# braun-steven/DAFNe

Hardware: AMD Instinct MI355X
Metric: images/sec on 1024x1024 DOTA tiles, R101-FPN (higher is better)
Workload: dtype bf16; 1 GPU; DOTA-1.0 1024x1024 R101-FPN bf16, batch 8 per GPU (per-GPU shard of configs[2]; the model BASELINE.json's metric names), uint8 tiles resident in HBM -> detections; per_gpu_batch=8, global_batch=8, classes=15, parallelism=dp1 (independent images, RCCL gather of detections), mode=pipelined

## Files before the change

### dafne_amd/_lib.py

```python
import ctypes
import os

_HERE = os.path.dirname(os.path.abspath(__file__))
LIB_PATH = os.environ.get("DAFNE_AMD_LIB") or os.path.join(_HERE, "libdafne_amd.so")
_lib = None

c_void_p = ctypes.c_void_p
c_int = ctypes.c_int
c_i64 = ctypes.c_int64
c_size_t = ctypes.c_size_t
c_double = ctypes.c_double
c_float = ctypes.c_float
c_u32 = ctypes.c_uint32
c_i32 = ctypes.c_int32


class LevelDesc(ctypes.Structure):
    _fields_ = [("d_logits", c_void_p), ("d_delta", c_void_p), ("d_center", c_void_p),
                ("d_ctrness", c_void_p), ("logits_ps", c_i32), ("delta_ps", c_i32),
                ("center_ps", c_i32), ("ctrness_ps", c_i32), ("H", c_i32), ("W", c_i32), ("stride", c_i32),
                ("scale", c_float)]


class DecodeParams(ctypes.Structure):
# ... 95 lines not shown
    "dafne_conv2d_wr_workspace_bytes": (c_size_t, [ctypes.POINTER(ConvParams), ctypes.POINTER(ConvSeg)]),
    "dafne_conv2d_wr_hip": (c_int, [ctypes.POINTER(ConvParams), ctypes.POINTER(ConvSeg), c_void_p, c_void_p, c_size_t, c_void_p]),
    "dafne_bottleneck_body_scratch_bytes": (c_size_t, []),
    "dafne_bottleneck_body_hip": (c_int, [c_void_p, c_void_p, c_void_p, c_void_p, c_void_p, c_void_p, c_int, c_int, c_int,
                                          c_void_p, c_void_p, c_void_p, c_size_t, c_void_p]),
    "dafne_bottleneck_tail_head_hip": (c_int, [c_void_p, c_void_p, c_void_p, c_void_p, c_void_p, c_int, c_int, c_int,
                                               c_void_p, c_void_p, c_void_p]),
    "dafne_bottleneck_tail_head_narrow_hip": (c_int, [c_void_p, c_void_p, c_void_p, c_void_p, c_void_p, c_int, c_int, c_int,
                                                      c_void_p, c_void_p, c_void_p]),
    "dafne_bottleneck_tail_head_mid_hip": (c_int, [c_void_p, c_void_p, c_void_p, c_void_p, c_void_p, c_int, c_int, c_int,
                                                   c_void_p, c_void_p, c_void_p]),
    "dafne_bottleneck_proj_tail_head_narrow_hip": (c_int, [c_void_p, c_void_p, c_void_p, c_void_p, c_void_p, c_void_p, c_int,
                                                           c_int, c_int, c_void_p, c_void_p, c_void_p]),
    "dafne_bottleneck_block_narrow_scratch_bytes": (c_size_t, []),
    "dafne_bottleneck_block_narrow_hip": (c_int, [c_void_p] * 7 + [c_int, c_int, c_int, c_void_p, c_void_p, c_void_p, c_size_t, c_void_p]),
    "dafne_bottleneck_block_mid_scratch_bytes": (c_size_t, []),
    "dafne_bottleneck_block_mid_hip": (c_int, [c_void_p] * 6 + [c_int, c_int, c_int, c_void_p, c_void_p, c_void_p, c_size_t, c_void_p]),
    "dafne_stem_pool_hip": (c_int, [c_void_p, c_void_p, c_void_p, c_int, c_int, c_int, c_void_p, c_void_p]),
    "dafne_stem_pool_conv1_hip": (c_int, [c_void_p, c_void_p, c_void_p, c_void_p, c_void_p, c_int, c_int, c_int, c_void_p, c_void_p,
                                          c_void_p]),
    "dafne_maxpool3x3s2_nhwc_bf16_hip": (c_int, [c_void_p, c_void_p, c_int, c_int, c_int, c_int, c_void_p]),
    "dafne_groupnorm_relu_nhwc_bf16_hip": (c_int, [ctypes.POINTER(GnSeg), c_int, c_int, c_int, c_void_p, c_void_p,
                                                   c_void_p, c_void_p, c_float, c_void_p]),
    "dafne_relu_copy_bf16_hip": (c_int, [c_void_p, c_void_p, c_i64, c_void_p]),
    "dafne_scene_tiles_workspace_bytes": (c_size_t, [c_int]),
    "dafne_scene_tiles_u8_hip": (c_int, [ctypes.POINTER(SceneTile), c_int, c_int, c_void_p, c_void_p, c_size_t, c_void_p]),
    "dafne_scene_merge_workspace_bytes": (c_size_t, [c_int, c_int]),
    "dafne_scene_merge_rows_hip": (c_int, [c_void_p, c_void_p, c_int, c_int, c_void_p, c_int, c_int, ctypes.c_uint64, c_int,
                                           c_int, c_void_p, c_void_p, c_void_p, c_void_p, c_size_t, c_void_p]),
    "dafne_scene_views_workspace_bytes": (c_size_t, [ctypes.POINTER(ViewSrc), c_int, c_int, c_int]),
# ... 48 lines not shown
```

### dafne_amd/csrc/abi.hip

```cpp
#include "common.h"

namespace dafne {
char* err_buf() {
    static thread_local char buf[512] = {0};
    return buf;
}
}

extern "C" {
int dafne_abi_version(void) { return 145; }
const char* dafne_last_error(void) { return dafne::err_buf(); }
}
```

### dafne_amd/csrc/conv_wr.hip

```cpp
#include <type_traits>

#include "common.h"

namespace {

typedef __attribute__((ext_vector_type(8))) __bf16 bf16x8;
typedef __attribute__((ext_vector_type(16))) float f32x16;
typedef __attribute__((ext_vector_type(4))) float f32x4;
typedef __attribute__((ext_vector_type(4))) unsigned u32x4;
typedef __attribute__((ext_vector_type(2))) unsigned u32x2;
typedef __attribute__((address_space(1))) void gvoid;
typedef __attribute__((address_space(3))) void lvoid;

constexpr int kPx = 128, kCT = 256;
constexpr int kNominalBatch = 8;
constexpr int kNW = 8, kNT = 512;
constexpr int kPF = kPx / 32;
constexpr int kStage = kPx * 128;
constexpr int kNS = 3;
constexpr int kSlabY = kPx * 128;
constexpr int kOffFlag = 4 * kSlabY;
constexpr int kSmemTotal = kOffFlag + 64;
constexpr int kSlabBytes = kPx * kCT * 4;
constexpr int kCounterBytes = 64 * 1024;
// ... 25 lines not shown
    typedef __attribute__((ext_vector_type(2))) float f32x2;
    typedef __attribute__((ext_vector_type(2))) __bf16 bf16x2;
    f32x2 v = {a, b};
    bf16x2 r = __builtin_convertvector(v, bf16x2);
    return __builtin_bit_cast(unsigned, r);
}

template <int I, int N, class F>
__device__ __forceinline__ void static_for(F&& f) {
    if constexpr (I < N) {
        f(std::integral_constant<int, I>{});
        static_for<I + 1, N>(f);
    }
}

__global__ void __launch_bounds__(512, 2) conv_wr_kernel(WrDev P) {
    extern __shared__ __attribute__((aligned(16))) char lds[];
    const int tid = threadIdx.x;
    const int lane = tid & 63;
    const int wave = __builtin_amdgcn_readfirstlane(tid >> 6);
    const int frow = lane & 31, half = lane >> 5;
    const unsigned lds_base = (unsigned)(size_t)(__attribute__((address_space(3))) char*)lds;

    const int id = xcd_remap(blockIdx.x, gridDim.x);
    const int slice = id % P.S;
    const int t = id / P.S;
    const int pt = t % P.ptiles, ct = t / P.ptiles;
    const int k_begin = (int)((long long)slice * P.nsteps / P.S);
    const int k_end = (int)((long long)(slice + 1) * P.nsteps / P.S);
    const int nst = k_end - k_begin;
// ... 82 lines not shown
        const int nxt = cur == kNS - 1 ? 0 : cur + 1;
        static_for<0, 4>([&](auto SS) {
            constexpr int s = decltype(SS)::value;
            if constexpr (s < 3) {
                asm volatile("s_waitcnt vmcnt(11)" : "+v"(ar[par * 4 + s]) :: "memory");
                bread(cur, s + 1, bfr[(s + 1) & 1]);
                asm volatile("s_waitcnt lgkmcnt(4)" : "+v"(bfr[s & 1][0]), "+v"(bfr[s & 1][1]), "+v"(bfr[s & 1][2]), "+v"(bfr[s & 1][3]) :: "memory");
            } else {
                asm volatile("s_waitcnt vmcnt(9)" : "+v"(ar[par * 4 + s]) :: "memory");
                asm volatile("s_waitcnt lgkmcnt(0)" : "+v"(bfr[1][0]), "+v"(bfr[1][1]), "+v"(bfr[1][2]), "+v"(bfr[1][3]) :: "memory");
                __builtin_amdgcn_sched_barrier(0);
                __builtin_amdgcn_s_barrier();
                __builtin_amdgcn_sched_barrier(0);
                bread(nxt, 0, bfr[0]);
            }
            __builtin_amdgcn_sched_barrier(0);
#pragma unroll
            for (int b = 0; b < kPF; b++) acc[b] = __builtin_amdgcn_mfma_f32_32x32x16_bf16(ar[par * 4 + s], bfr[s & 1][b], acc[b], 0, 0, 0);
            __builtin_amdgcn_sched_barrier(0);
            issue_W(4 * i + 8 + s, ar[par * 4 + s]);
            if constexpr (s == 3) issue_P(i + 3, cur);
        });
        cur = nxt;
    };
    int i = 0;
    for (; i + 1 < nst; i += 2) {
        step(i, std::integral_constant<int, 0>{});
        step(i + 1, std::integral_constant<int, 1>{});
    }
    if (i < nst) step(i, std::integral_constant<int, 0>{});
// ... 94 lines not shown
            int img, oy, ox;
            out_coords(px, img, oy, ox);
            char* dst = P.out + (((size_t)(img * (P.Hout + 2) + oy + 1) * (P.Wout + 2) + ox + 1) * P.Cout + ct * kCT) * 2 + q * 16;
#pragma unroll
            for (int sl = 0; sl < 4; sl++) {
                const u32x4 v = *(const u32x4*)(lds + sl * kSlabY + px * 128 + ((q ^ ((px >> 1) & 7)) * 16));
                *(u32x4*)(dst + sl * 128) = v;
            }
        }
    }
}

int wr_build(WrDev& D, const dafne_conv_params* prm, const dafne_conv_seg* segs, const char** why) {
    *why = nullptr;
    if (!prm || !segs) { *why = "null argument"; return 0; }
    const unsigned allowed = DAFNE_CONV_RELU | DAFNE_CONV_RESIDUAL | DAFNE_CONV_UPSAMPLE_ADD | DAFNE_CONV_EXCLUSIVE;
    if (prm->n_segs != 1) { *why = "one segment"; return 0; }
    if (prm->flags & ~allowed) { *why = "flags"; return 0; }
    if ((prm->flags & DAFNE_CONV_RESIDUAL) && (prm->flags & DAFNE_CONV_UPSAMPLE_ADD)) { *why = "residual and top-down add"; return 0; }
    if (!((prm->KH == 1 && prm->KW == 1 && prm->pad == 0) || (prm->KH == 3 && prm->KW == 3 && prm->pad == 1))) { *why = "1x1 p0 or 3x3 p1"; return 0; }
    if (prm->stride != 1 && prm->stride != 2) { *why = "stride"; return 0; }
    if (prm->Cin < 64 || prm->Cin % 64 || prm->Cout < kCT || prm->Cout % kCT) { *why = "Cin % 64, Cout % 256"; return 0; }
    if (!prm->d_bias) { *why = "bias"; return 0; }
    const dafne_conv_seg& S = segs[0];
    if (prm->n_images < 1 || S.Hout < 1 || S.Wout < 1 || (long long)S.Hout * S.Wout > (1 << 20)) { *why = "size"; return 0; }
    if (S.Hout != (S.Hin + 2 * prm->pad - prm->KH) / prm->stride + 1 || S.Wout != (S.Win + 2 * prm->pad - prm->KW) / prm->stride + 1) { *why = "geometry"; return 0; }
    if ((prm->flags & DAFNE_CONV_UPSAMPLE_ADD) && ((S.Hout & 1) || (S.Wout & 1))) { *why = "top-down add on an odd map"; return 0; }
    const long long in_bytes = (long long)prm->n_images * (S.Hin + 2) * (S.Win + 2) * prm->Cin * 2;
    const long long total = (long long)prm->n_images * S.Hout * S.Wout;
    if (in_bytes > 0xffffffffll || total > (1ll << 21)) { *why = "too large"; return 0; }
    D.in = (const char*)S.d_in; D.out = (char*)S.d_out; D.res = (const char*)S.d_res;
// ... 43 lines not shown
}

int dafne_conv2d_wr_hip(const dafne_conv_params* prm, const dafne_conv_seg* segs, const void* d_wfrag, void* d_workspace,
                        size_t workspace_bytes, void* stream) {
    WrDev D;
    const char* why;
    if (!wr_build(D, prm, segs, &why)) return dafne::fail(why && why[0] == 'n' ? DAFNE_E_INVALID : DAFNE_E_UNSUPPORTED, "conv2d_wr: %s", why ? why : "?");
    if (!d_wfrag || !D.in || !D.out) return dafne::fail(DAFNE_E_INVALID, "conv2d_wr: null argument");
    if ((D.flags & (DAFNE_CONV_RESIDUAL | DAFNE_CONV_UPSAMPLE_ADD)) && !D.res) return dafne::fail(DAFNE_E_INVALID, "conv2d_wr: residual flag without d_res");
    const size_t tiles = (size_t)D.ptiles * D.ctiles;
    const size_t need = D.S > 1 ? (size_t)kCounterBytes + tiles * D.S * (size_t)kSlabBytes : 0;
    if (D.S > 1 && (!d_workspace || workspace_bytes < need)) return dafne::fail(DAFNE_E_WORKSPACE, "conv2d_wr: workspace %zu < %zu", workspace_bytes, need);
    D.wf = (const char*)d_wfrag;
    D.counters = (int*)d_workspace;
    D.slabs = (char*)d_workspace + kCounterBytes;
    DAFNE_MAX_LDS_ONCE(kSmemTotal, (const void*)conv_wr_kernel);
    hipLaunchKernelGGL(conv_wr_kernel, dim3((unsigned)(tiles * D.S)), dim3(kNT), kSmemTotal, (hipStream_t)stream, D);
    return dafne::check_launch("conv_wr");
}

}
```

### dafne_amd/engine.py

```python
import ctypes
import os

import torch

from . import _lib

BF16 = torch.bfloat16
STAGE_BLOCKS = {50: (3, 4, 6, 3), 101: (3, 4, 23, 3)}

F_RELU, F_RES, F_UP, F_F32, F_GN, F_GNIN, F_GNFIN, F_EXCL = 1, 2, 4, 8, 16, 32, 64, 128
F_FRAG16 = 256


class Act:

    __slots__ = ("t", "n", "h", "w", "c")

    def __init__(self, n, h, w, c, device):
        self.t = torch.zeros(n, h + 2, w + 2, c, dtype=BF16, device=device)
        self.n, self.h, self.w, self.c = n, h, w, c

    def nchw_float(self):
        return self.t[:, 1:-1, 1:-1, :].permute(0, 3, 1, 2).float().contiguous()

    @staticmethod
    def from_nchw(x):
# ... 492 lines not shown
                if calib is not None:
                    self.calls.append(AmaxProbe(calib, key, [tin]))
                elif key in act_q8:
                    fp8 = (q8[1] / act_q8[key], act_q8[key])
            c = ConvCall(q8[0] if fp8 else wgt, bias, cin, cout, k, stride, pad, flags,
                         [(tin.t, o.t, res.t if res is not None else None, tin.h, tin.w, ho, wo)], n, fp8=fp8,
                         shared_gpu=self.shared_gpu)
            if (fp8 is None and wr_on and wr_takes(k, stride, cin, cout, WR_NOMINAL_BATCH * ho * wo) and bias is not None
                    and L.dafne_conv2d_wr_ok(ctypes.byref(c.prm), c.segs)):
                if key + ".wr" not in P:
                    P[key + ".wr"] = pack_conv_frag(wgt)
                w = WrCall(c, P[key + ".wr"], self.wr_ws)
                self.calls.append(w)
                self.flops += w.flops
                return o
            if fp8 is None and k == 3 and cin == 256 and use_rp_kernel() and c.kernel_id() == 6 and c.rp_ok():
                f16 = rp_frag16()
                fkey = key + (".frag16" if f16 else ".frag")
                if fkey not in P:
                    P[fkey] = pack_rp(wgt)[0]
                c = ConvCall(wgt, bias, cin, cout, k, stride, pad, flags,
                             [(tin.t, o.t, None, tin.h, tin.w, ho, wo)], n, wfrag=P[fkey], shared_gpu=self.shared_gpu, frag16=f16)
            self.calls.append(c)
            self.flops += c.flops
            return o

        self.stem_in = torch.zeros(n, h + 6, w + 6, 4, dtype=BF16, device=device)
        wgt, bias = P["stem"]
        x = pool.get(n, h // 4, w // 4, 64)
        stem_flops = 2 * n * (h // 2) * (w // 2) * 64 * 7 * 7 * 3
# ... 25 lines not shown
            self.calls.append(FnCall(L.dafne_maxpool3x3s2_nhwc_bf16_hip,
                                     (_lib.ptr(stem_out.t), _lib.ptr(x.t), n, h // 2, w // 2, 64),
                                     (stem_out, x), "maxpool"))
            pool.put(stem_out)

        feats = {}
        fuse_b2b = os.environ.get("DAFNE_FUSE_B2B", "1") != "0"
        fuse_narrow = fuse_b2b and os.environ.get("DAFNE_FUSE_B2B_NARROW", "1") != "0"
        fuse_mid = fuse_b2b and os.environ.get("DAFNE_FUSE_B2B_MID", "1") != "0"
        fuse_bneck = fuse_b2b and os.environ.get("DAFNE_FUSE_BNECK", "1") != "0"
        bneck_scratch = None
        blk_scratch = None
        blk_mid_scratch = None
        fuse_blk_mid = fuse_mid and os.environ.get("DAFNE_FUSE_BLK_MID", "1") != "0"
        fuse_blk_narrow = fuse_narrow and os.environ.get("DAFNE_FUSE_BLK_NARROW", "1") != "0"
        for si, nb in enumerate(STAGE_BLOCKS[depth]):
            y1_next = stem_y1 if si == 0 else None
            for b in range(nb):
                p = "res%d.%d." % (si + 2, b)
                stride = 2 if (b == 0 and si > 0) else 1
                w3, b3 = P[p + "conv3"]
                nxt = "res%d.%d.conv1" % (si + 2, b + 1)
                proj_fused = (fuse_narrow and b == 0 and stride == 1 and nb > 1 and tuple(w3.shape) == (256, 64)
                              and tuple(P[p + "shortcut"][0].shape) == (256, 64) and tuple(P[nxt][0].shape) == (64, 256))
                if b == 0:
                    sc = None if proj_fused else conv(p + "shortcut", x, 1, stride, 0, 0)
                else:
                    sc = x
                if y1_next is not None:
                    y1, y1_next = y1_next, None
                else:
                    y1 = conv(p + "conv1", x, 1, stride, 0, F_RELU)
                w2, b2 = P[p + "conv2"]
                q8_2 = P.get(p + "conv2.fp8")
                bn_head = b + 1 < nb
                body_fused = (fuse_bneck and tuple(w3.shape) == (1024, 256) and (not bn_head or tuple(P[nxt][0].shape) == (256, 1024))
                              and (bn_head or os.environ.get("DAFNE_FUSE_BNECK_LAST", "1") != "0")
                              and tuple(w2.shape) == (256, 2304) and y1.c == 256
                              and not (q8_2 is not None and (calib is not None or (p + "conv2") in act_q8)))
                if body_fused:
                    w1, b1 = P[nxt] if bn_head else (torch.zeros(256, 1024, dtype=BF16, device=w2.device), None)
                    key = p + "bneck"
                    if key not in P:
                        P[key] = pack_bneck(w2, w3, w1)
                    if bneck_scratch is None:
                        bneck_scratch = torch.empty(L.dafne_bottleneck_body_scratch_bytes(), dtype=torch.uint8, device=device)
                    inpl = res_dead(sc, x, b)
                    y3 = sc if inpl else pool.get(n, y1.h, y1.w, 1024)
                    y1_next = pool.get(n, y1.h, y1.w, 256) if bn_head else None
                    fl = 2 * n * y1.h * y1.w * (256 * 2304 + 256 * 1024 + (1024 * 256 if bn_head else 0))
                    nb_ = n * y1.h * y1.w * (256 + 1024 + 1024 + (256 if bn_head else 0)) * 2 + (256 * 2304 + 2 * 1024 * 256) * 2
                    self.calls.append(FnCall(L.dafne_bottleneck_body_hip,
                                             (_lib.ptr(y1.t), _lib.ptr(sc.t), _lib.ptr(P[key]), _lib.ptr(b2), _lib.ptr(b3), _lib.ptr(b1),
                                              n, y1.h, y1.w, _lib.ptr(y3.t), _lib.ptr(y1_next.t) if bn_head else None, _lib.ptr(bneck_scratch),
                                              bneck_scratch.numel()),
                                             (y1, sc, P[key], b2, b3, b1, y3, y1_next, bneck_scratch),
                                             "conv_bneck" if bn_head else "conv_bneck_last", flops=fl, nbytes=nb_))
                    self.flops += fl
                    pool.put(y1)
                    if b == 0 and sc is not None and sc is not y3:
                        pool.put(sc)
                    if x is not y3 and not any(x is f for k, f in feats.items() if k != "res2"):
                        pool.put(x)
                    x = y3
                    continue
                if (fuse_blk_narrow and tuple(w2.shape) == (64, 576) and tuple(w3.shape) == (256, 64) and y1.c == 64 and stride == 1
                        and (b > 0 or proj_fused) and (b + 1 >= nb or tuple(P[nxt][0].shape) == (64, 256))):
                    head = b + 1 < nb
                    proj = b == 0
                    w1, b1 = P[nxt] if head else (None, None)
                    wsc, bsc = P[p + "shortcut"] if proj else (None, None)
                    key = p + "blk"
                    if key not in P:
                        P[key] = pack_blk_narrow(w2, w3, w1, wsc)
                    if blk_scratch is None:
                        blk_scratch = torch.empty(L.dafne_bottleneck_block_narrow_scratch_bytes(), dtype=torch.uint8, device=device)
                    src = x if proj else sc
                    inpl = (not proj) and res_dead(sc, x, b)
                    y3 = sc if inpl else pool.get(n, y1.h, y1.w, 256)
                    y1_next = pool.get(n, y1.h, y1.w, 64) if head else None
                    px = n * y1.h * y1.w
                    fl = 2 * px * (64 * 576 + 64 * 256 + (256 * 64 if head else 0) + (64 * 256 if proj else 0))
                    nb_ = px * (64 + (64 if proj else 256) + 256 + (64 if head else 0)) * 2 + P[key].numel() * 2
                    self.calls.append(FnCall(L.dafne_bottleneck_block_narrow_hip,
                                             (_lib.ptr(y1.t), _lib.ptr(src.t), _lib.ptr(P[key]), _lib.ptr(b2), _lib.ptr(b3), _lib.ptr(bsc),
                                              _lib.ptr(b1), n, y1.h, y1.w, _lib.ptr(y3.t), _lib.ptr(y1_next.t) if head else None,
                                              _lib.ptr(blk_scratch), blk_scratch.numel()),
                                             (y1, src, P[key], b2, b3, bsc, b1, y3, y1_next, blk_scratch),
                                             "conv_blk_narrow" + ("_proj" if proj else "") + ("" if head else "_last"), flops=fl, nbytes=nb_))
                    self.flops += fl
                    pool.put(y1)
                    if x is not y3 and not any(x is f for k, f in feats.items() if k != "res2"):
                        pool.put(x)
                    x = y3
                    continue
                if (fuse_blk_mid and tuple(w2.shape) == (128, 1152) and tuple(w3.shape) == (512, 128) and y1.c == 128
                        and (b + 1 >= nb or tuple(P[nxt][0].shape) == (128, 512))):
                    head = b + 1 < nb
                    w1, b1 = P[nxt] if head else (None, None)
                    key = p + "blk"
                    if key not in P:
                        P[key] = pack_blk_mid(w2, w3, w1)
                    if blk_mid_scratch is None:
                        blk_mid_scratch = torch.empty(L.dafne_bottleneck_block_mid_scratch_bytes(), dtype=torch.uint8, device=device)
                    inpl = res_dead(sc, x, b)
                    y3 = sc if inpl else pool.get(n, y1.h, y1.w, 512)
                    y1_next = pool.get(n, y1.h, y1.w, 128) if head else None
                    px = n * y1.h * y1.w
                    fl = 2 * px * (128 * 1152 + 128 * 512 + (512 * 128 if head else 0))
                    nb_ = px * (128 + 512 + 512 + (128 if head else 0)) * 2 + P[key].numel() * 2
                    self.calls.append(FnCall(L.dafne_bottleneck_block_mid_hip,
                                             (_lib.ptr(y1.t), _lib.ptr(sc.t), _lib.ptr(P[key]), _lib.ptr(b2), _lib.ptr(b3), _lib.ptr(b1),
                                              n, y1.h, y1.w, _lib.ptr(y3.t), _lib.ptr(y1_next.t) if head else None,
                                              _lib.ptr(blk_mid_scratch), blk_mid_scratch.numel()),
                                             (y1, sc, P[key], b2, b3, b1, y3, y1_next, blk_mid_scratch),
                                             "conv_blk_mid" + ("" if head else "_last"), flops=fl, nbytes=nb_))
                    self.flops += fl
                    pool.put(y1)
                    if b == 0 and sc is not None and sc is not y3:
                        pool.put(sc)
                    if x is not y3 and not any(x is f for k, f in feats.items() if k != "res2"):
                        pool.put(x)
                    x = y3
                    continue
                y2 = conv(p + "conv2", y1, 3, 1, 1, F_RELU)
                pool.put(y1)
                if proj_fused:
                    w1, b1 = P[nxt]
                    wsc, bsc = P[p + "shortcut"]
                    key = p + "b2b"
                    if key not in P:
                        P[key] = pack_b2b_narrow(w3, w1, wsc)
                    y3 = pool.get(n, y2.h, y2.w, 256)
                    y1_next = pool.get(n, y2.h, y2.w, 64)
                    fl = 2 * n * y2.h * y2.w * (64 * 256 * 2 + 256 * 64)
                    nb_ = n * y2.h * y2.w * (64 + 64 + 256 + 64) * 2 + 3 * 256 * 64 * 2
# ... 37 lines not shown
                        P[key] = pack_b2b_narrow(w3, w1)
                    y3 = pool.get(n, y2.h, y2.w, 256)
                    y1_next = pool.get(n, y2.h, y2.w, 64)
                    fl = 2 * n * y2.h * y2.w * (64 * 256 + 256 * 64)
                    nb_ = n * y2.h * y2.w * (64 + 256 + 256 + 64) * 2 + 2 * 256 * 64 * 2
                    self.calls.append(FnCall(L.dafne_bottleneck_tail_head_narrow_hip,
                                             (_lib.ptr(y2.t), _lib.ptr(sc.t), _lib.ptr(P[key]), _lib.ptr(b3), _lib.ptr(b1),
                                              n, y2.h, y2.w, _lib.ptr(y3.t), _lib.ptr(y1_next.t)),
                                             (y2, sc, P[key], b3, b1, y3, y1_next), "conv_b2b_narrow", flops=fl, nbytes=nb_))
                    self.flops += fl
                else:
                    y3 = conv(p + "conv3", y2, 1, 1, 0, F_RELU | F_RES, res=sc)
                pool.put(y2)
                if b == 0 and sc is not None:
                    pool.put(sc)
                if not any(x is f for k, f in feats.items() if k != "res2"):
                    pool.put(x)
                x = y3
            feats["res%d" % (si + 2)] = x
        self.stage_feats = feats
        prev = None
        outs = {}
        for lvl in (5, 4, 3):
            f = feats["res%d" % lvl]
            lat = conv("fpn_lateral%d" % lvl, f, 1, 1, 0, F_UP if prev is not None else 0, res=prev)
            outs["p%d" % lvl] = conv("fpn_output%d" % lvl, lat, 3, 1, 1, 0)
            prev = lat
        p6 = conv("p6", outs["p5"], 3, 2, 1, 0)
        p6r = pool.get(n, p6.h, p6.w, p6.c)
        self.calls.append(FnCall(L.dafne_relu_copy_bf16_hip, (_lib.ptr(p6.t), _lib.ptr(p6r.t), p6.t.numel()),
                                 (p6, p6r), "relu_copy"))
        p7 = conv("p7", p6r, 3, 2, 1, 0)
        outs["p6"], outs["p7"] = p6, p7
        self.features = [outs[k] for k in ("p3", "p4", "p5", "p6", "p7")]
        self.head_start = len(self.calls)
        self.head = HeadPlan(weights, self.features, num_classes, device, pool, self, head_outputs) if with_head else None
        if any(isinstance(c, WrCall) for c in self.calls):
            self.wr_ws.tensor()

    def run(self, stream=None):
        if self.graph is not None and stream is None:
            self.graph.replay()
            return
        stream = stream if stream is not None else _lib.current_stream()
        for c in self.calls:
            c(stream)

# ... 319 lines not shown
```

### include/dafne_amd.h

```cpp
#ifndef DAFNE_AMD_H
#define DAFNE_AMD_H

#include <stddef.h>
#include <stdint.h>

#ifdef __cplusplus
extern "C" {
#endif

#define DAFNE_OK 0
#define DAFNE_E_INVALID 1
#define DAFNE_E_WORKSPACE 2
#define DAFNE_E_HIP 3
#define DAFNE_E_UNSUPPORTED 4

int dafne_abi_version(void);
const char* dafne_last_error(void);

int dafne_poly_iou_pairs_hip(const double* d_p, const double* d_q, int64_t n,
                             double* d_out, void* stream);

size_t dafne_poly_nms_f64_workspace_bytes(int n_images, int m_cap);
int dafne_poly_nms_f64_batched_hip(const double* d_dets9, const int32_t* d_counts, int n_images, int m_cap,
                                   double thresh, int strict_hbb, int64_t* d_keep, int32_t* d_num_keep,
// ... 48 lines not shown
                                const int32_t* d_levels, const float* d_hbox,
                                const int64_t* d_keep, const int32_t* d_num_keep,
                                const float* d_sizes, int do_postprocess, int n_images, int m_cap,
                                int k_cap, float* d_out, int32_t* d_out_counts, void* stream);

#define DAFNE_CONV_RELU 1u
#define DAFNE_CONV_RESIDUAL 2u
#define DAFNE_CONV_UPSAMPLE_ADD 4u
#define DAFNE_CONV_OUT_F32 8u
#define DAFNE_CONV_GN_STATS 16u
#define DAFNE_CONV_GN_INPUT 32u
#define DAFNE_CONV_GN_FINALIZE 64u
#define DAFNE_CONV_EXCLUSIVE 128u

#define DAFNE_CONV_FRAG16 256u

typedef struct dafne_conv_seg {
    const void* d_in;
    void* d_out;
    const void* d_res;
    int32_t Hin, Win, Hout, Wout;
} dafne_conv_seg;

typedef struct dafne_conv_params {
    int32_t n_images, n_segs;
    int32_t Cin, Cout, KH, KW, stride, pad;
    uint32_t flags;
    const void* d_weight;
    const float* d_bias;
    float* d_gn_partial;
// ... 46 lines not shown
                              const float* d_bias3, const float* d_bias1, int n_images, int H, int W, void* d_out,
                              void* d_next, void* d_scratch, size_t scratch_bytes, void* stream);
int dafne_bottleneck_tail_head_narrow_hip(const void* d_in, const void* d_res, const void* d_wfrag, const float* d_bias3,
                                          const float* d_bias1, int n_images, int H, int W, void* d_out, void* d_next,
                                          void* stream);
int dafne_bottleneck_tail_head_mid_hip(const void* d_in, const void* d_res, const void* d_wfrag, const float* d_bias3,
                                       const float* d_bias1, int n_images, int H, int W, void* d_out, void* d_next,
                                       void* stream);
int dafne_bottleneck_proj_tail_head_narrow_hip(const void* d_in, const void* d_x0, const void* d_wfrag, const float* d_bias3,
                                               const float* d_bias_sc, const float* d_bias1, int n_images, int H, int W,
                                               void* d_out, void* d_next, void* stream);
size_t dafne_bottleneck_block_narrow_scratch_bytes(void);
int dafne_bottleneck_block_narrow_hip(const void* d_in, const void* d_res, const void* d_wfrag, const float* d_bias2,
                                      const float* d_bias3, const float* d_bias_sc, const float* d_bias1, int n_images, int H, int W,
                                      void* d_out, void* d_next, void* d_scratch, size_t scratch_bytes, void* stream);
size_t dafne_bottleneck_block_mid_scratch_bytes(void);
int dafne_bottleneck_block_mid_hip(const void* d_in, const void* d_res, const void* d_wfrag, const float* d_bias2,
                                   const float* d_bias3, const float* d_bias1, int n_images, int H, int W, void* d_out,
                                   void* d_next, void* d_scratch, size_t scratch_bytes, void* stream);
int dafne_stem_pool_hip(const void* d_in, const void* d_weight, const float* d_bias, int n_images, int H, int W,
                        void* d_out, void* stream);
int dafne_stem_pool_conv1_hip(const void* d_in, const void* d_weight, const float* d_bias, const void* d_w1, const float* d_b1,
                              int n_images, int H, int W, void* d_out, void* d_out1, void* stream);
int dafne_maxpool3x3s2_nhwc_bf16_hip(const void* d_in, void* d_out, int n_images, int Hin, int Win,
                                     int C, void* stream);

typedef struct dafne_gn_seg {
    void* d_x;
    int32_t H, W;
    int32_t tile0, tiles_per_img;
// ... 62 lines not shown
```

Baseline: 1466 images/sec.

## Fuse last res2 block with stride-2 output and fold p6 ReLU into p7 conv

Adds a new fused kernel for the last res2 bottleneck block. It computes conv2 and conv3 plus the residual only at the stride-2 pixel positions that res3's conv1 and shortcut consume, writing a compacted output so res3 block 0 can use stride 1. This is possible because res2 is not an FPN input, and it cuts conv3 work and output traffic by about 4x for that block. Separately, the conv_wr kernel gains a RELU_INPUT template variant that rectifies the input fragments on load, removing the separate relu_copy pass between p6 and p7. The risks are extra code paths and changed buffer-lifetime bookkeeping (only res3, res4 and res5 are now protected from reuse).

Measured after the change: 1486 images/sec, median of 6. 1.01x the previous value.

```diff
diff --git a/dafne_amd/_lib.py b/dafne_amd/_lib.py
--- a/dafne_amd/_lib.py
+++ b/dafne_amd/_lib.py
@@ -133,6 +133,8 @@
                                                            c_int, c_int, c_void_p, c_void_p, c_void_p]),
     "dafne_bottleneck_block_narrow_scratch_bytes": (c_size_t, []),
     "dafne_bottleneck_block_narrow_hip": (c_int, [c_void_p] * 7 + [c_int, c_int, c_int, c_void_p, c_void_p, c_void_p, c_size_t, c_void_p]),
+    "dafne_bottleneck_block_narrow_s2_scratch_bytes": (c_size_t, []),
+    "dafne_bottleneck_block_narrow_s2_hip": (c_int, [c_void_p] * 5 + [c_int, c_int, c_int, c_void_p, c_void_p, c_size_t, c_void_p]),
     "dafne_bottleneck_block_mid_scratch_bytes": (c_size_t, []),
     "dafne_bottleneck_block_mid_hip": (c_int, [c_void_p] * 6 + [c_int, c_int, c_int, c_void_p, c_void_p, c_void_p, c_size_t, c_void_p]),
     "dafne_stem_pool_hip": (c_int, [c_void_p, c_void_p, c_void_p, c_int, c_int, c_int, c_void_p, c_void_p]),
diff --git a/dafne_amd/csrc/abi.hip b/dafne_amd/csrc/abi.hip
--- a/dafne_amd/csrc/abi.hip
+++ b/dafne_amd/csrc/abi.hip
@@ -8,6 +8,6 @@
 }
 
 extern "C" {
-int dafne_abi_version(void) { return 145; }
+int dafne_abi_version(void) { return 146; }
 const char* dafne_last_error(void) { return dafne::err_buf(); }
 }
diff --git a/dafne_amd/csrc/conv_blk_narrow_s2.hip b/dafne_amd/csrc/conv_blk_narrow_s2.hip
--- /dev/null
+++ b/dafne_amd/csrc/conv_blk_narrow_s2.hip
@@ -0,0 +1,292 @@
+#include <stdlib.h>
+
+#include "common.h"
+
+namespace {
+
+typedef __attribute__((ext_vector_type(8))) __bf16 bf16x8;
+typedef __attribute__((ext_vector_type(16))) float f32x16;
+typedef __attribute__((ext_vector_type(4))) unsigned u32x4;
+typedef __attribute__((ext_vector_type(2))) unsigned u32x2;
+typedef __attribute__((address_space(1))) void gvoid;
+typedef __attribute__((address_space(3))) void lvoid;
+
+constexpr int kTH = 2, kTW = 32, kPx = kTH * kTW;
+constexpr int kPC = 2 * kTW + 1, kPR = 2 * kTH + 1;
+constexpr int kPPieces = (kPR * kPC + 7) / 8;
+constexpr int kPPerWave = (kPPieces + 7) / 8;
+constexpr int kPatch = kPPieces * 1024;
+constexpr int kSlab = kPx * 128;
+constexpr int kCM = 64, kCB = 256;
+constexpr int kStepsA = 36;
+constexpr int kW2Bytes = 2 * kStepsA * 1024;
+constexpr int kOffW2 = 0;
+constexpr int kOffPatch = kOffW2 + kW2Bytes;
+constexpr int kOffT = kOffPatch + kPatch;
+constexpr int kOffY = kOffT + kSlab;
+constexpr int kOffBias = kOffY + 4 * kSlab;
+constexpr int kSmemTotal = kOffBias + 4096;
+static_assert((kCM + kCB) * 4 <= 4096 && kSmemTotal <= 160 * 1024, "LDS budget");
+constexpr int kNW = 8, kNT = 512;
+constexpr int kDumpBytes = kPx * kCB * 2;
+constexpr int kWfA3 = kW2Bytes;
+
+struct BlkS2Dev {
+    const char* in;
+    const char* res;
+    const char* wf;
+    const float* b2;
+    const float* b3;
+    char* out;
+    char* dump;
+    int N, H, W, Ho, Wo, tiles_x, tiles_per_img, tiles;
+    unsigned max_pix;
+};
+
+__device__ __forceinline__ unsigned pack_bf16(float a, float b) {
+    typedef __attribute__((ext_vector_type(2))) float f32x2;
+    typedef __attribute__((ext_vector_type(2))) __bf16 bf16x2;
+    f32x2 v = {a, b};
+    bf16x2 r = __builtin_convertvector(v, bf16x2);
+    return __builtin_bit_cast(unsigned, r);
+}
+
+__global__ void __launch_bounds__(512, 2) conv_blk_narrow_s2_kernel(BlkS2Dev P) {
+    extern __shared__ __attribute__((aligned(16))) char lds[];
+    const int tid = threadIdx.x;
+    const int lane = tid & 63;
+    const int wave = __builtin_amdgcn_readfirstlane(tid >> 6);
+    const int frow = lane & 31, half = lane >> 5;
+    const unsigned lds_base = (unsigned)(size_t)(__attribute__((address_space(3))) char*)lds;
+    const int Wp = P.W + 2, Wop = P.Wo + 2;
+    const int G = gridDim.x;
+    const int my_tiles = (P.tiles - (int)blockIdx.x + G - 1) / G;
+
+    struct TileXY { int img, row0, col0; };
+    auto tile_xy = [&](int t) {
+        TileXY r;
+        r.img = t / P.tiles_per_img;
+        const int rem = t - r.img * P.tiles_per_img;
+        const int ty = rem / P.tiles_x;
+        r.row0 = ty * kTH;
+        r.col0 = (rem - ty * P.tiles_x) * kTW;
+        return r;
+    };
+    auto x_index = [&](const TileXY& T, int px) {
+        int r = T.row0 + (px >> 5), c = T.col0 + (px & 31);
+        r = r < P.Ho ? r : P.Ho - 1;
+        c = c < P.Wo ? c : P.Wo - 1;
+        return (unsigned)((T.img * (P.H + 2) + 2 * r + 1) * Wp + 2 * c + 1);
+    };
+    auto y_index = [&](const TileXY& T, int px) {
+        return (unsigned)((T.img * (P.Ho + 2) + T.row0 + (px >> 5) + 1) * Wop + T.col0 + (px & 31) + 1);
+    };
+    auto pix_valid = [&](const TileXY& T, int px) { return T.row0 + (px >> 5) < P.Ho && T.col0 + (px & 31) < P.Wo; };
+
+#pragma unroll
+    for (int i = 0; i < 9; i++)
+        __builtin_amdgcn_global_load_lds((gvoid*)(P.wf + (size_t)(wave * 9 + i) * 1024 + lane * 16), (lvoid*)(lds + kOffW2 + (wave * 9 + i) * 1024), 16, 0, 0);
+    const int cq = wave & 3, pf = wave >> 2;
+    const int ct = wave & 1, pt = (wave >> 1) & 1;
+    bf16x8 a3[8];
+    {
+#pragma unroll
+        for (int h = 0; h < 2; h++)
+#pragma unroll
+            for (int s = 0; s < 4; s++) {
+                const char* w3 = P.wf + kWfA3 + (size_t)((h * 4 + cq) * 4 + s) * 1024 + lane * 16;
+                asm volatile("global_load_dwordx4 %0, %1, off" : "=v"(a3[h * 4 + s]) : "v"(w3) : "memory");
+            }
+        float* lb = (float*)(lds + kOffBias);
+        if (tid < kCM) lb[tid] = P.b2[tid];
+        if (tid < kCB) lb[kCM + tid] = P.b3[tid];
+    }
+
+    auto issue_patch = [&](const TileXY& T) {
+#pragma unroll
+        for (int ii = 0; ii < kPPerWave; ii++) {
+            int pc = wave + kNW * ii;
+            pc = pc < kPPieces ? pc : kPPieces - 1;
+            int ln = lane;
+            asm volatile("" : "+v"(ln));
+            const int pp = pc * 8 + (ln >> 3);
+            const int p = (pp * 1009) >> 16;
+            const int q = pp - p * kPC;
+            unsigned g = (unsigned)((T.img * (P.H + 2) + 2 * T.row0 + p) * Wp + 2 * T.col0 + q);
+            g = g < P.max_pix ? g : P.max_pix;
+            __builtin_amdgcn_global_load_lds((gvoid*)(P.in + (size_t)g * (kCM * 2) + (unsigned)(((ln & 7) ^ ((q >> 1) & 7)) * 16)),
+                                             (lvoid*)(lds + kOffPatch + pc * 1024), 16, 0, 0);
+        }
+    };
+    u32x4 rr[4];
+#pragma unroll
+    for (int i = 0; i < 4; i++) rr[i] = u32x4{0u, 0u, 0u, 0u};
+    auto issue_x = [&](const TileXY& T) {
+#pragma unroll
+        for (int i = 0; i < 4; i++) {
+            int idx = tid + kNT * i;
+            asm volatile("" : "+v"(idx));
+            const char* src = P.res + (size_t)x_index(T, idx >> 5) * (kCB * 2) + (idx & 31) * 16;
+            asm volatile("global_load_dwordx4 %0, %1, off nt" : "+v"(rr[i]) : "v"(src) : "memory");
+        }
+    };
+
+    unsigned bs[4];
+#pragma unroll
+    for (int s = 0; s < 4; s++) bs[s] = (unsigned)(frow * 128 + (((2 * s + half) ^ ((frow >> 1) & 7)) * 16));
+    auto barrier = [&]() {
+        __builtin_amdgcn_sched_barrier(0);
+        asm volatile("s_waitcnt lgkmcnt(0)" ::: "memory");
+        __builtin_amdgcn_s_barrier();
+        __builtin_amdgcn_sched_barrier(0);
+    };
+    const float* lbias = (const float*)(lds + kOffBias);
+
+    if (my_tiles > 0) {
+        const TileXY T0 = tile_xy((int)blockIdx.x);
+        issue_patch(T0);
+        issue_x(T0);
+    }
+    asm volatile("s_waitcnt vmcnt(0)" ::: "memory");
+#pragma unroll
+    for (int s = 0; s < 8; s++) asm volatile("" : "+v"(a3[s]));
+
+    for (int kk = 0; kk < my_tiles; kk++) {
+        const int t = (int)blockIdx.x + kk * G;
+        const TileXY T = tile_xy(t);
+        const TileXY Tn = tile_xy(kk + 1 < my_tiles ? t + G : t);
+        if (kk > 0) asm volatile("s_waitcnt vmcnt(4)" ::: "memory");
+#pragma unroll
+        for (int i = 0; i < 4; i++) {
+            asm volatile("" : "+v"(rr[i]));
+            const int idx = tid + kNT * i;
+            const int px = idx >> 5, j = idx & 31;
+            const unsigned ad = lds_base + (unsigned)(kOffY + (j >> 3) * kSlab + px * 128 + (((j & 7) ^ ((px >> 1) & 7)) * 16));
+            asm volatile("ds_write_b128 %0, %1" ::"v"(ad), "v"(rr[i]) : "memory");
+        }
+        barrier();
+        if (wave < 4) {
+            f32x16 acc;
+#pragma unroll
+            for (int k = 0; k < 16; k++) acc[k] = 0.f;
+            int fr = frow;
+            asm volatile("" : "+v"(fr));
+            const char* wa = lds + kOffW2 + ct * kStepsA * 1024 + lane * 16;
+#pragma unroll
+            for (int kh = 0; kh < 3; kh++)
+#pragma unroll
+                for (int kw = 0; kw < 3; kw++) {
+                    const int q = kw + 2 * fr;
+                    const char* pb = lds + kOffPatch + ((2 * pt + kh) * kPC + q) * 128;
+                    const int sw = (q >> 1) & 7;
+                    bf16x8 af[4], bf[4];
+#pragma unroll
+                    for (int s = 0; s < 4; s++) {
+                        af[s] = *(const bf16x8*)(wa + ((kh * 3 + kw) * 4 + s) * 1024);
+                        bf[s] = *(const bf16x8*)(pb + (((2 * s + half) ^ sw) * 16));
+                    }
+#pragma unroll
+                    for (int s = 0; s < 4; s++) acc = __builtin_amdgcn_mfma_f32_32x32x16_bf16(af[s], bf[s], acc, 0, 0, 0);
+                }
+            const int px = pt * 32 + frow;
+            const unsigned tb = lds_base + (unsigned)(kOffT + px * 128 + 8 * half);
+#pragma unroll
+            for (int g = 0; g < 4; g++) {
+                const float* bp = lbias + ct * 32 + 8 * g + 4 * half;
+                const float v0 = fmaxf(acc[4 * g] + bp[0], 0.f), v1 = fmaxf(acc[4 * g + 1] + bp[1], 0.f);
+                const float v2 = fmaxf(acc[4 * g + 2] + bp[2], 0.f), v3 = fmaxf(acc[4 * g + 3] + bp[3], 0.f);
+                u32x2 pk;
+                pk.x = pack_bf16(v0, v1);
+                pk.y = pack_bf16(v2, v3);
+                const unsigned ad = tb + (unsigned)((((ct * 4 + g) ^ ((px >> 1) & 7))) * 16);
+                asm volatile("ds_write_b64 %0, %1" ::"v"(ad), "v"(pk) : "memory");
+            }
+        }
+        barrier();
+        issue_patch(Tn);
+        issue_x(Tn);
+        __builtin_amdgcn_sched_barrier(0);
+#pragma unroll
+        for (int h = 0; h < 2; h++) {
+            f32x16 acc1;
+#pragma unroll
+            for (int k = 0; k < 16; k++) acc1[k] = 0.f;
+            bf16x8 bfr[4];
+#pragma unroll
+            for (int s = 0; s < 4; s++) bfr[s] = *(const bf16x8*)(lds + kOffT + pf * 4096 + bs[s]);
+#pragma unroll
+            for (int s = 0; s < 4; s++) acc1 = __builtin_amdgcn_mfma_f32_32x32x16_bf16(a3[h * 4 + s], bfr[s], acc1, 0, 0, 0);
+            {
+                typedef __attribute__((ext_vector_type(4))) float f32x4;
+                typedef __attribute__((ext_vector_type(2))) float f32x2;
+                const unsigned ebase = lds_base + (unsigned)(kOffY + (2 * h + (cq >> 1)) * kSlab + pf * 4096 + frow * 128 + 8 * half);
+#pragma unroll
+                for (int g = 0; g < 4; g++) {
+                    const unsigned ead = ebase + (unsigned)(((((cq & 1) * 4 + g) ^ ((frow >> 1) & 7))) * 16);
+                    const f32x4 bv = *(const f32x4*)(lbias + kCM + h * 128 + cq * 32 + 8 * g + 4 * half);
+                    u32x2 r;
+                    asm volatile("ds_read_b64 %0, %1\n\ts_waitcnt lgkmcnt(0)" : "=&v"(r) : "v"(ead) : "memory");
+                    const f32x2 blo = {bv[0], bv[1]}, bhi = {bv[2], bv[3]};
+                    const f32x2 rlo = {__uint_as_float(r.x << 16), __uint_as_float(r.x & 0xffff0000u)};
+                    const f32x2 rhi = {__uint_as_float(r.y << 16), __uint_as_float(r.y & 0xffff0000u)};
+                    const f32x2 alo = {acc1[4 * g], acc1[4 * g + 1]}, ahi = {acc1[4 * g + 2], acc1[4 * g + 3]};
+                    const f32x2 vlo = alo + blo + rlo, vhi = ahi + bhi + rhi;
+                    r.x = pack_bf16(fmaxf(vlo[0], 0.f), fmaxf(vlo[1], 0.f));
+                    r.y = pack_bf16(fmaxf(vhi[0], 0.f), fmaxf(vhi[1], 0.f));
+                    asm volatile("ds_write_b64 %1, %0" ::"v"(r), "v"(ead) : "memory");
+                }
+            }
+        }
+        barrier();
+#pragma unroll
+        for (int i = 0; i < 4; i++) {
+            int idx = tid + kNT * i;
+            asm volatile("" : "+v"(idx));
+            const int px = idx >> 5, j = idx & 31;
+            const u32x4 v = *(const u32x4*)(lds + kOffY + (j >> 3) * kSlab + px * 128 + (((j & 7) ^ ((px >> 1) & 7)) * 16));
+            char* a = P.out + (size_t)y_index(T, px) * (kCB * 2);
+            char* d = P.dump + (size_t)px * (kCB * 2);
+            a = pix_valid(T, px) ? a : d;
+            __builtin_nontemporal_store(v, (u32x4*)(a + j * 16));
+        }
+        barrier();
+        __builtin_amdgcn_sched_barrier(0);
+    }
+    asm volatile("s_waitcnt vmcnt(0)" ::: "memory");
+}
+
+}
+
+extern "C" {
+
+size_t dafne_bottleneck_block_narrow_s2_scratch_bytes(void) { return (size_t)kDumpBytes; }
+
+int dafne_bottleneck_block_narrow_s2_hip(const void* d_in, const void* d_res, const void* d_wfrag, const float* d_bias2,
+                                         const float* d_bias3, int n_images, int H, int W, void* d_out, void* d_scratch,
+                                         size_t scratch_bytes, void* stream) {
+    if (!d_in || !d_res || !d_wfrag || !d_bias2 || !d_bias3 || !d_out || !d_scratch)
+        return dafne::fail(DAFNE_E_INVALID, "bottleneck_block_narrow_s2: null argument");
+    if (n_images < 1 || H < 1 || W < 1 || (long long)H * W > (1 << 20)) return dafne::fail(DAFNE_E_INVALID, "bottleneck_block_narrow_s2: bad size");
+    if (scratch_bytes < (size_t)kDumpBytes) return dafne::fail(DAFNE_E_WORKSPACE, "bottleneck_block_narrow_s2: scratch %zu < %d", scratch_bytes, kDumpBytes);
+    BlkS2Dev D;
+    D.in = (const char*)d_in; D.res = (const char*)d_res; D.wf = (const char*)d_wfrag;
+    D.b2 = d_bias2; D.b3 = d_bias3;
+    D.out = (char*)d_out; D.dump = (char*)d_scratch;
+    D.N = n_images; D.H = H; D.W = W;
+    D.Ho = (H + 1) / 2; D.Wo = (W + 1) / 2;
+    D.tiles_x = (D.Wo + kTW - 1) / kTW;
+    D.tiles_per_img = D.tiles_x * ((D.Ho + kTH - 1) / kTH);
+    const long long tiles = (long long)D.tiles_per_img * n_images;
+    const long long pix = (long long)n_images * (H + 2) * (W + 2);
+    if (tiles > (1ll << 24) || pix * (kCB * 2) > 0xffffffffll) return dafne::fail(DAFNE_E_UNSUPPORTED, "bottleneck_block_narrow_s2: too large");
+    D.tiles = (int)tiles;
+    D.max_pix = (unsigned)(pix - 1);
+    DAFNE_MAX_LDS_ONCE(kSmemTotal, (const void*)conv_blk_narrow_s2_kernel);
+    int n_cu = 0;
+    if (int rc = dafne::device_cus(&n_cu)) return rc;
+    const int grid = D.tiles < n_cu ? D.tiles : n_cu;
+    hipLaunchKernelGGL(conv_blk_narrow_s2_kernel, dim3(grid), dim3(kNT), kSmemTotal, (hipStream_t)stream, D);
+    return dafne::check_launch("conv_blk_narrow_s2");
+}
+
+}
diff --git a/dafne_amd/csrc/conv_wr.hip b/dafne_amd/csrc/conv_wr.hip
--- a/dafne_amd/csrc/conv_wr.hip
+++ b/dafne_amd/csrc/conv_wr.hip
@@ -5,6 +5,7 @@
 namespace {
 
 typedef __attribute__((ext_vector_type(8))) __bf16 bf16x8;
+typedef __attribute__((ext_vector_type(8))) short s16x8;
 typedef __attribute__((ext_vector_type(16))) float f32x16;
 typedef __attribute__((ext_vector_type(4))) float f32x4;
 typedef __attribute__((ext_vector_type(4))) unsigned u32x4;
@@ -63,6 +64,7 @@
     }
 }
 
+template <bool RELU_IN>
 __global__ void __launch_bounds__(512, 2) conv_wr_kernel(WrDev P) {
     extern __shared__ __attribute__((aligned(16))) char lds[];
     const int tid = threadIdx.x;
@@ -175,6 +177,13 @@
                 __builtin_amdgcn_sched_barrier(0);
                 bread(nxt, 0, bfr[0]);
             }
+            if constexpr (RELU_IN) {
+#pragma unroll
+                for (int b = 0; b < kPF; b++) {
+                    const s16x8 v = __builtin_bit_cast(s16x8, bfr[s & 1][b]);
+                    bfr[s & 1][b] = __builtin_bit_cast(bf16x8, __builtin_elementwise_max(v, s16x8{}));
+                }
+            }
             __builtin_amdgcn_sched_barrier(0);
 #pragma unroll
             for (int b = 0; b < kPF; b++) acc[b] = __builtin_amdgcn_mfma_f32_32x32x16_bf16(ar[par * 4 + s], bfr[s & 1][b], acc[b], 0, 0, 0);
@@ -299,7 +308,7 @@
 int wr_build(WrDev& D, const dafne_conv_params* prm, const dafne_conv_seg* segs, const char** why) {
     *why = nullptr;
     if (!prm || !segs) { *why = "null argument"; return 0; }
-    const unsigned allowed = DAFNE_CONV_RELU | DAFNE_CONV_RESIDUAL | DAFNE_CONV_UPSAMPLE_ADD | DAFNE_CONV_EXCLUSIVE;
+    const unsigned allowed = DAFNE_CONV_RELU | DAFNE_CONV_RESIDUAL | DAFNE_CONV_UPSAMPLE_ADD | DAFNE_CONV_EXCLUSIVE | DAFNE_CONV_RELU_INPUT;
     if (prm->n_segs != 1) { *why = "one segment"; return 0; }
     if (prm->flags & ~allowed) { *why = "flags"; return 0; }
     if ((prm->flags & DAFNE_CONV_RESIDUAL) && (prm->flags & DAFNE_CONV_UPSAMPLE_ADD)) { *why = "residual and top-down add"; return 0; }
@@ -373,8 +382,9 @@
     D.wf = (const char*)d_wfrag;
     D.counters = (int*)d_workspace;
     D.slabs = (char*)d_workspace + kCounterBytes;
-    DAFNE_MAX_LDS_ONCE(kSmemTotal, (const void*)conv_wr_kernel);
-    hipLaunchKernelGGL(conv_wr_kernel, dim3((unsigned)(tiles * D.S)), dim3(kNT), kSmemTotal, (hipStream_t)stream, D);
+    DAFNE_MAX_LDS_ONCE(kSmemTotal, (const void*)conv_wr_kernel<false>, (const void*)conv_wr_kernel<true>);
+    if (D.flags & DAFNE_CONV_RELU_INPUT) hipLaunchKernelGGL(conv_wr_kernel<true>, dim3((unsigned)(tiles * D.S)), dim3(kNT), kSmemTotal, (hipStream_t)stream, D);
+    else hipLaunchKernelGGL(conv_wr_kernel<false>, dim3((unsigned)(tiles * D.S)), dim3(kNT), kSmemTotal, (hipStream_t)stream, D);
     return dafne::check_launch("conv_wr");
 }
 
diff --git a/dafne_amd/engine.py b/dafne_amd/engine.py
--- a/dafne_amd/engine.py
+++ b/dafne_amd/engine.py
@@ -10,6 +10,8 @@
 
 F_RELU, F_RES, F_UP, F_F32, F_GN, F_GNIN, F_GNFIN, F_EXCL = 1, 2, 4, 8, 16, 32, 64, 128
 F_FRAG16 = 256
+F_RELU_INPUT = 512
+FPN_IN_FEATURES = ("res3", "res4", "res5")
 
 
 class Act:
@@ -532,6 +534,7 @@
                 self.calls.append(w)
                 self.flops += w.flops
                 return o
+            assert not (flags & F_RELU_INPUT), "only conv_wr rectifies its input on load (the caller checks wr_takes)"
             if fp8 is None and k == 3 and cin == 256 and use_rp_kernel() and c.kernel_id() == 6 and c.rp_ok():
                 f16 = rp_frag16()
                 fkey = key + (".frag16" if f16 else ".frag")
@@ -587,6 +590,9 @@
         blk_mid_scratch = None
         fuse_blk_mid = fuse_mid and os.environ.get("DAFNE_FUSE_BLK_MID", "1") != "0"
         fuse_blk_narrow = fuse_narrow and os.environ.get("DAFNE_FUSE_BLK_NARROW", "1") != "0"
+        tail_s2 = os.environ.get("DAFNE_RES2_TAIL_S2", "1") != "0"
+        blk_s2_scratch = None
+        x_compact = False
         for si, nb in enumerate(STAGE_BLOCKS[depth]):
             y1_next = stem_y1 if si == 0 else None
             for b in range(nb):
@@ -596,14 +602,16 @@
                 nxt = "res%d.%d.conv1" % (si + 2, b + 1)
                 proj_fused = (fuse_narrow and b == 0 and stride == 1 and nb > 1 and tuple(w3.shape) == (256, 64)
                               and tuple(P[p + "shortcut"][0].shape) == (256, 64) and tuple(P[nxt][0].shape) == (64, 256))
+                in_stride = 1 if (b == 0 and x_compact) else stride
                 if b == 0:
-                    sc = None if proj_fused else conv(p + "shortcut", x, 1, stride, 0, 0)
+                    sc = None if proj_fused else conv(p + "shortcut", x, 1, in_stride, 0, 0)
                 else:
                     sc = x
                 if y1_next is not None:
                     y1, y1_next = y1_next, None
                 else:
-                    y1 = conv(p + "conv1", x, 1, stride, 0, F_RELU)
+                    y1 = conv(p + "conv1", x, 1, in_stride, 0, F_RELU)
+                x_compact = False
                 w2, b2 = P[p + "conv2"]
                 q8_2 = P.get(p + "conv2.fp8")
                 bn_head = b + 1 < nb
@@ -633,7 +641,7 @@
                     pool.put(y1)
                     if b == 0 and sc is not None and sc is not y3:
                         pool.put(sc)
-                    if x is not y3 and not any(x is f for k, f in feats.items() if k != "res2"):
+                    if x is not y3 and not any(x is f for k, f in feats.items() if k in FPN_IN_FEATURES):
                         pool.put(x)
                     x = y3
                     continue
@@ -649,6 +657,26 @@
                     if blk_scratch is None:
                         blk_scratch = torch.empty(L.dafne_bottleneck_block_narrow_scratch_bytes(), dtype=torch.uint8, device=device)
                     src = x if proj else sc
+                    nx0 = "res%d.0." % (si + 3)
+                    if (tail_s2 and calib is None and not head and not proj and si + 1 < len(STAGE_BLOCKS[depth])
+                            and "res%d" % (si + 2) not in FPN_IN_FEATURES
+                            and tuple(P[nx0 + "conv1"][0].shape)[1:] == (256,) and tuple(P[nx0 + "shortcut"][0].shape)[1:] == (256,)):
+                        if blk_s2_scratch is None:
+                            blk_s2_scratch = torch.empty(L.dafne_bottleneck_block_narrow_s2_scratch_bytes(), dtype=torch.uint8, device=device)
+                        ho, wo = (y1.h + 1) // 2, (y1.w + 1) // 2
+                        y3 = pool.get(n, ho, wo, 256)
+                        fl = 2 * n * ho * wo * (64 * 576 + 64 * 256)
+                        nb_ = n * (y1.h * y1.w * 64 + ho * wo * (256 + 256)) * 2 + (64 * 576 + 256 * 64) * 2
+                        self.calls.append(FnCall(L.dafne_bottleneck_block_narrow_s2_hip,
+                                                 (_lib.ptr(y1.t), _lib.ptr(src.t), _lib.ptr(P[key]), _lib.ptr(b2), _lib.ptr(b3), n, y1.h, y1.w,
+                                                  _lib.ptr(y3.t), _lib.ptr(blk_s2_scratch), blk_s2_scratch.numel()),
+                                                 (y1, src, P[key], b2, b3, y3, blk_s2_scratch), "conv_blk_narrow_s2", flops=fl, nbytes=nb_))
+                        self.flops += fl
+                        pool.put(y1)
+                        pool.put(x)
+                        x = y3
+                        x_compact = True
+                        continue
                     inpl = (not proj) and res_dead(sc, x, b)
                     y3 = sc if inpl else pool.get(n, y1.h, y1.w, 256)
                     y1_next = pool.get(n, y1.h, y1.w, 64) if head else None
@@ -663,7 +691,7 @@
                                              "conv_blk_narrow" + ("_proj" if proj else "") + ("" if head else "_last"), flops=fl, nbytes=nb_))
                     self.flops += fl
                     pool.put(y1)
-                    if x is not y3 and not any(x is f for k, f in feats.items() if k != "res2"):
+                    if x is not y3 and not any(x is f for k, f in feats.items() if k in FPN_IN_FEATURES):
                         pool.put(x)
                     x = y3
                     continue
@@ -692,7 +720,7 @@
                     pool.put(y1)
                     if b == 0 and sc is not None and sc is not y3:
                         pool.put(sc)
-                    if x is not y3 and not any(x is f for k, f in feats.items() if k != "res2"):
+                    if x is not y3 and not any(x is f for k, f in feats.items() if k in FPN_IN_FEATURES):
                         pool.put(x)
                     x = y3
                     continue
@@ -760,7 +788,7 @@
                 pool.put(y2)
                 if b == 0 and sc is not None:
                     pool.put(sc)
-                if not any(x is f for k, f in feats.items() if k != "res2"):
+                if not any(x is f for k, f in feats.items() if k in FPN_IN_FEATURES):
                     pool.put(x)
                 x = y3
             feats["res%d" % (si + 2)] = x
@@ -773,10 +801,16 @@
             outs["p%d" % lvl] = conv("fpn_output%d" % lvl, lat, 3, 1, 1, 0)
             prev = lat
         p6 = conv("p6", outs["p5"], 3, 2, 1, 0)
-        p6r = pool.get(n, p6.h, p6.w, p6.c)
-        self.calls.append(FnCall(L.dafne_relu_copy_bf16_hip, (_lib.ptr(p6.t), _lib.ptr(p6r.t), p6.t.numel()),
-                                 (p6, p6r), "relu_copy"))
-        p7 = conv("p7", p6r, 3, 2, 1, 0)
+        w7, b7 = P["p7"]
+        ho7, wo7 = conv_out_hw(p6.h, p6.w, 3, 2, 1)
+        if (os.environ.get("DAFNE_P7_RELU_IN", "1") != "0" and wr_on and b7 is not None
+                and wr_takes(3, 2, p6.c, w7.shape[0], WR_NOMINAL_BATCH * ho7 * wo7)):
+            p7 = conv("p7", p6, 3, 2, 1, F_RELU_INPUT)
+        else:
+            p6r = pool.get(n, p6.h, p6.w, p6.c)
+            self.calls.append(FnCall(L.dafne_relu_copy_bf16_hip, (_lib.ptr(p6.t), _lib.ptr(p6r.t), p6.t.numel()),
+                                     (p6, p6r), "relu_copy"))
+            p7 = conv("p7", p6r, 3, 2, 1, 0)
         outs["p6"], outs["p7"] = p6, p7
         self.features = [outs[k] for k in ("p3", "p4", "p5", "p6", "p7")]
         self.head_start = len(self.calls)
diff --git a/include/dafne_amd.h b/include/dafne_amd.h
--- a/include/dafne_amd.h
+++ b/include/dafne_amd.h
@@ -86,6 +86,7 @@
 #define DAFNE_CONV_EXCLUSIVE 128u
 
 #define DAFNE_CONV_FRAG16 256u
+#define DAFNE_CONV_RELU_INPUT 512u
 
 typedef struct dafne_conv_seg {
     const void* d_in;
@@ -162,6 +163,10 @@
 int dafne_bottleneck_block_narrow_hip(const void* d_in, const void* d_res, const void* d_wfrag, const float* d_bias2,
                                       const float* d_bias3, const float* d_bias_sc, const float* d_bias1, int n_images, int H, int W,
                                       void* d_out, void* d_next, void* d_scratch, size_t scratch_bytes, void* stream);
+size_t dafne_bottleneck_block_narrow_s2_scratch_bytes(void);
+int dafne_bottleneck_block_narrow_s2_hip(const void* d_in, const void* d_res, const void* d_wfrag, const float* d_bias2,
+                                         const float* d_bias3, int n_images, int H, int W, void* d_out, void* d_scratch,
+                                         size_t scratch_bytes, void* stream);
 size_t dafne_bottleneck_block_mid_scratch_bytes(void);
 int dafne_bottleneck_block_mid_hip(const void* d_in, const void* d_res, const void* d_wfrag, const float* d_bias2,
                                    const float* d_bias3, const float* d_bias1, int n_images, int H, int W, void* d_out,
```
